# waicool20/BoofCV

Hardware: AMD Instinct MI355X
Metric: 1080p frames/sec detect+describe+associate (higher is better)
Workload: dtype f32 detect / f64 describe / associate: fp16 MFMA candidate filter + exact fp64 re-score; 1 GPU; batch of 256 1920x1080 GrayF32 per GPU: Fast-Hessian detect + SURF-64 (stable) describe + greedy L2 associate with the next frame; batch_per_gpu=256, width=1920, height=1080, ranks_seen=1

## Files before the change

boofcv_amd/csrc/assoc_mfma.hip:

```cpp
#include "common.h"
#include <cfloat>
#include <cmath>
#include <cstring>
#include <algorithm>

typedef float f32x16 __attribute__((ext_vector_type(16)));
typedef _Float16 h16x8 __attribute__((ext_vector_type(8)));

struct AssocProblem {
	int srcOff, ns, dstOff, nd;
	int rowBase, colBase;
};
struct AssocBlock {
	int p, row0, row1, col0, col1;
};
struct AssocCand {
	int p, i, j, pad;
	double score;
};

#define C16 1.03e-3f
#define ABS16 2.0e-5f
#define BIG16 60000.0f
#define ROW_CHUNKS 9

__device__ __forceinline__ void waveSyncLds() {
	__builtin_amdgcn_fence(__ATOMIC_RELEASE, "wavefront");
	__builtin_amdgcn_wave_barrier();
	__builtin_amdgcn_fence(__ATOMIC_ACQUIRE, "wavefront");
}

__host__ __device__ __forceinline__ int scaleExp(float maxN) {
	if (!(maxN > 0.0f)) return 0;
	int e;
	(void)frexpf(maxN, &e);
	return (e + 1) >> 1;
}
__host__ __device__ __forceinline__ bool scaleHolds(float maxN, int q) {
	if (!(maxN > 0.0f)) return true;
	int e;
	(void)frexpf(maxN, &e);
	return e >= 2 * q - 3 && e <= 2 * q;
}
__host__ __device__ __forceinline__ bool assocDegenerate(const int* flags, int cap) {
	float maxN;
	memcpy(&maxN, &flags[1], 4);
	return flags[0] != 0 || flags[2] > cap || !scaleHolds(maxN, flags[3]);
}

#define PREP_ROWS 8
__global__ __launch_bounds__(256) void k_assoc_norms(const double* __restrict__ D, long long rows, float* __restrict__ nrm, int* __restrict__ flags) {
	const long long row0 = (((long long)blockIdx.x * 256 + threadIdx.x) >> 4) * PREP_ROWS;
	const int part = threadIdx.x & 15;
	if (row0 >= rows) return;
	double2 v0[PREP_ROWS], v1[PREP_ROWS];
#pragma unroll
	for (int q = 0; q < PREP_ROWS; q++) {
		const long long row = min(row0 + q, rows - 1);
		const double2* src = (const double2*)(D + row * 64 + 4 * part);
		v0[q] = src[0]; v1[q] = src[1];
	}
#pragma unroll
	for (int q = 0; q < PREP_ROWS; q++) {
		double s = (v0[q].x * v0[q].x + v0[q].y * v0[q].y) + (v1[q].x * v1[q].x + v1[q].y * v1[q].y);
#pragma unroll
		for (int o = 8; o >= 1; o >>= 1) s += __shfl_xor(s, o, 64);
		if (part == 0 && row0 + q < rows) {
			const float n = (float)s;
			const float nUp = n * (1.0f + 4.0f * 5.9604644775390625e-08f);
			nrm[row0 + q] = nUp;
			if (!(s < 1e30)) atomicOr(&flags[0], 1);
			else if (__float_as_int(nUp) > __hip_atomic_load(&flags[1], __ATOMIC_RELAXED, __HIP_MEMORY_SCOPE_AGENT)) atomicMax(&flags[1], __float_as_int(nUp));
		}
	}
}

typedef _Float16 h16x4 __attribute__((ext_vector_type(4)));
__global__ __launch_bounds__(256) void k_assoc_half(const double* __restrict__ D, long long rows, float* __restrict__ nrm, int* __restrict__ flags,
													  _Float16* __restrict__ Hrow) {
	const long long row0 = (((long long)blockIdx.x * 256 + threadIdx.x) >> 4) * PREP_ROWS;
	const int part = threadIdx.x & 15;
	if (row0 >= rows) return;
	const int q_ = scaleExp(__int_as_float(flags[1]));
	if (blockIdx.x == 0 && threadIdx.x == 0) flags[3] = q_;
	double2 v0[PREP_ROWS], v1[PREP_ROWS];
#pragma unroll
	for (int q = 0; q < PREP_ROWS; q++) {
		const long long row = min(row0 + q, rows - 1);
		const double2* src = (const double2*)(D + row * 64 + 4 * part);
		v0[q] = src[0]; v1[q] = src[1];
	}
#pragma unroll
	for (int q = 0; q < PREP_ROWS; q++) {
		const long long row = row0 + q;
		if (row >= rows) break;
		_Float16* out = Hrow + row * (ROW_CHUNKS * 8);
		const h16x4 hv = {(_Float16)(float)ldexp(v0[q].x, -q_), (_Float16)(float)ldexp(v0[q].y, -q_), (_Float16)(float)ldexp(v1[q].x, -q_),
						  (_Float16)(float)ldexp(v1[q].y, -q_)};
		*(h16x4*)(out + 4 * part) = hv;
		if (part == 0) {
			const float n = ldexpf(nrm[row], -2 * q_);
			const _Float16 hi = (_Float16)n;
			const _Float16 lo = (_Float16)(n - (float)hi);
			const h16x8 e = {hi, lo, (_Float16)1.0f, (_Float16)1.0f, (_Float16)1.0f, (_Float16)0.0f, (_Float16)0.0f, (_Float16)0.0f};
			*(h16x8*)(out + 64) = e;
			nrm[row] = n;
		}
	}
}

__global__ __launch_bounds__(256) void k_assoc_prep_hinted(const double* __restrict__ D, long long rows, int q_, float* __restrict__ nrm, int* __restrict__ flags,
															 _Float16* __restrict__ Hrow) {
	const long long row0 = (((long long)blockIdx.x * 256 + threadIdx.x) >> 4) * PREP_ROWS;
	const int part = threadIdx.x & 15;
	if (row0 >= rows) return;
	double2 v0[PREP_ROWS], v1[PREP_ROWS];
#pragma unroll
	for (int q = 0; q < PREP_ROWS; q++) {
		const long long row = min(row0 + q, rows - 1);
		const double2* src = (const double2*)(D + row * 64 + 4 * part);
		v0[q] = src[0]; v1[q] = src[1];
	}
#pragma unroll
	for (int q = 0; q < PREP_ROWS; q++) {
		double s = (v0[q].x * v0[q].x + v0[q].y * v0[q].y) + (v1[q].x * v1[q].x + v1[q].y * v1[q].y);
#pragma unroll
		for (int o = 8; o >= 1; o >>= 1) s += __shfl_xor(s, o, 64);
		const long long row = row0 + q;
		if (row >= rows) continue;
		_Float16* out = Hrow + row * (ROW_CHUNKS * 8);
		const h16x4 hv = {(_Float16)(float)ldexp(v0[q].x, -q_), (_Float16)(float)ldexp(v0[q].y, -q_), (_Float16)(float)ldexp(v1[q].x, -q_),
						  (_Float16)(float)ldexp(v1[q].y, -q_)};
		*(h16x4*)(out + 4 * part) = hv;
		if (part == 0) {
			const float nRaw = (float)s;
			const float nUp = nRaw * (1.0f + 4.0f * 5.9604644775390625e-08f);
			if (!(s < 1e30)) atomicOr(&flags[0], 1);
			else if (__float_as_int(nUp) > __hip_atomic_load(&flags[1], __ATOMIC_RELAXED, __HIP_MEMORY_SCOPE_AGENT)) atomicMax(&flags[1], __float_as_int(nUp));
			const float n = ldexpf(nUp, -2 * q_);
			const _Float16 hi = (_Float16)n;
			const _Float16 lo = (_Float16)(n - (float)hi);
			const h16x8 e = {hi, lo, (_Float16)1.0f, (_Float16)1.0f, (_Float16)1.0f, (_Float16)0.0f, (_Float16)0.0f, (_Float16)0.0f};
			*(h16x8*)(out + 64) = e;
			nrm[row] = n;
		}
	}
}

__global__ __launch_bounds__(256) void k_assoc_init(unsigned int* __restrict__ keys, unsigned long long* __restrict__ best, int* __restrict__ args, long long nk,
													  long long colTotal, int* __restrict__ flags, int q_, const uint4* __restrict__ tabSrc, uint4* __restrict__ tabDst,
													  long long tabWords) {
	const long long i = (long long)blockIdx.x * 256 + threadIdx.x;
	if (i < tabWords) tabDst[i] = tabSrc[i];
	if (i < 16) flags[i] = i == 3 ? q_ : 0;
	if (i >= nk) return;
	keys[i] = 0xFFFFFFFFu;
	best[i] = ~0ull;
	args[i] = -1;
	if (i < colTotal) args[nk + i] = 0;
}

struct MfmaArgs {
	const uint4* Hs;
	const uint4* Hd;
	const AssocProblem* probs;
	const AssocBlock* blocks;
	unsigned int* rowKey;
	unsigned int* colKey;
	const float* nrmS;
	const float* nrmD;
	const int* flags;
	AssocCand* cand;
	int* counter;
	int cap;
#ifdef BHIP_EXPERIMENTS
	int ablate;
#endif
};

#define CAND_LDS 256

__device__ __noinline__ void candSlow(AssocCand* cand, int* counter, int cap, int p, int rr, int col) {
	const int g = atomicAdd(counter, 1);
	if (g < cap) { AssocCand c; c.p = p; c.i = rr; c.j = col; c.pad = 0; c.score = 0; cand[g] = c; }
}
__device__ __forceinline__ void candAdd(const MfmaArgs& A, int2* buf, int* cnt, bool hit, int p, int rr, int col) {
	if (hit) {
		const int pos = atomicAdd(cnt, 1);
		if (pos < CAND_LDS) buf[pos] = make_int2(rr, col);
		else candSlow(A.cand, A.counter, A.cap, p, rr, col);
	}
}
__device__ __forceinline__ void candFlush(const MfmaArgs& A, const int2* buf, const int* cnt, int p, int lane) {
	waveSyncLds();
	const int n = min(*cnt, CAND_LDS);
	if (n == 0) return;
	int base = 0;
	if (lane == 0) base = atomicAdd(A.counter, n);
	base = __builtin_amdgcn_readfirstlane(base);
	for (int k = lane; k < n; k += 64) {
		if (base + k < A.cap) {
			const int2 v = buf[k];
			AssocCand c; c.p = p; c.i = v.x; c.j = v.y; c.pad = 0; c.score = 0;
			A.cand[base + k] = c;
		}
	}
}

__device__ __forceinline__ h16x8 asHalf8(uint4 v) { return __builtin_bit_cast(h16x8, v); }
__device__ __forceinline__ uint4 extChunk(float n0, float n1, float n2, float n3) {
	const h16x8 h = {(_Float16)n0, (_Float16)n1, (_Float16)n2, (_Float16)n3, (_Float16)1.0f, (_Float16)0.0f, (_Float16)0.0f, (_Float16)0.0f};
	return __builtin_bit_cast(uint4, h);
}

#ifndef BHIP_ASSOC_PEEL
#define BHIP_ASSOC_PEEL 1
#endif
#define STRIP_COLS 384
#define STRIP_TILES (STRIP_COLS / 32)
template <int PASS>
__global__ __launch_bounds__(256, 2) void k_assoc_mfma(MfmaArgs A) {
	__shared__ uint4 tileB[STRIP_TILES][10 * 33];
	__shared__ unsigned int colLds[STRIP_COLS];
	__shared__ float rowThrLds[PASS == 2 ? 4 : 1][64];
	__shared__ int2 candLds[PASS == 2 ? 4 : 1][PASS == 2 ? CAND_LDS : 1];
	__shared__ int candCnt[4];
	const AssocBlock B = A.blocks[blockIdx.x];
	if (B.col0 >= B.col1) return;
	const AssocProblem P = A.probs[B.p];
	const int tid = threadIdx.x;
	const int wave = __builtin_amdgcn_readfirstlane(tid >> 6), lane = tid & 63;
	const int r = lane & 31, h = lane >> 5;
	const int ncol = B.col1 - B.col0;
	const int ntile = (ncol + 31) >> 5;
	int2* candBuf = candLds[PASS == 2 ? wave : 0];
	int* candN = &candCnt[wave];
	if (lane == 0) *candN = 0;

	for (int g0 = tid; g0 < ntile * 32 * ROW_CHUNKS; g0 += 4 * 256) {
		uint4 v[4];
#pragma unroll
		for (int q = 0; q < 4; q++) {
			const int g = g0 + 256 * q;
			const int cl = g / ROW_CHUNKS, ch = g - cl * ROW_CHUNKS;
			if (g < ntile * 32 * ROW_CHUNKS && cl < ncol) {
				v[q] = A.Hd[(long long)(P.dstOff + B.col0 + cl) * ROW_CHUNKS + ch];
				if (ch == 8) { const unsigned int x = v[q].x; v[q].x = v[q].y; v[q].y = x; }
			} else {
				v[q] = ch == 8 ? extChunk(1.0f, 1.0f, BIG16, 0.0f) : make_uint4(0, 0, 0, 0);
			}
		}
#pragma unroll
		for (int q = 0; q < 4; q++) {
			const int g = g0 + 256 * q;
			const int cl = g / ROW_CHUNKS, ch = g - cl * ROW_CHUNKS;
			if (g < ntile * 32 * ROW_CHUNKS) tileB[cl >> 5][ch * 33 + (cl & 31)] = v[q];
		}
	}
	for (int g = tid; g < ntile * 32; g += 256) tileB[g >> 5][9 * 33 + (g & 31)] = make_uint4(0, 0, 0, 0);
	float maxN = 0.0f;
	if (PASS == 2) maxN = ldexpf(__int_as_float(A.flags[1]), -2 * A.flags[3]);
	for (int c = tid; c < ntile * 32; c += 256) {
		unsigned int v = 0xFFFFFFFFu;
		if (PASS == 2) {
			float thr = -INFINITY;
			if (c < ncol) {
				const float band = 2.0f * (C16 * (A.nrmD[P.dstOff + B.col0 + c] + maxN) + ABS16);
				thr = __uint_as_float(A.colKey[P.colBase + B.col0 + c]) + band;
			}
			v = __float_as_uint(thr);
		}
		colLds[c] = v;
	}
	__syncthreads();

	uint4 araw[2][5];
	auto loadA = [&](int rowT) {
#pragma unroll
		for (int t = 0; t < 2; t++) {
			const int row = rowT + 32 * t + r;
			if (row < B.row1) {
				const uint4* src = A.Hs + (long long)(P.srcOff + row) * ROW_CHUNKS;
#pragma unroll
				for (int s = 0; s < 4; s++) araw[t][s] = src[2 * s + h];
				araw[t][4] = h == 0 ? src[8] : make_uint4(0, 0, 0, 0);
			} else {
#pragma unroll
				for (int s = 0; s < 4; s++) araw[t][s] = make_uint4(0, 0, 0, 0);
				araw[t][4] = h == 0 ? extChunk(BIG16, 0.0f, 1.0f, 1.0f) : make_uint4(0, 0, 0, 0);
			}
		}
	};
	if (B.row0 + 64 * wave < B.row1) loadA(B.row0 + 64 * wave);
	for (int rowT = B.row0 + 64 * wave; rowT < B.row1; rowT += 256) {
		h16x8 a[2][5];
#pragma unroll
		for (int t = 0; t < 2; t++) {
#pragma unroll
			for (int s = 0; s < 4; s++) a[t][s] = asHalf8(araw[t][s]) * (_Float16)(-2.0f);
			a[t][4] = asHalf8(araw[t][4]);
		}
		if (rowT + 256 < B.row1 && !BHIP_ABLATE(A, 4)) loadA(rowT + 256);
		unsigned int rowM[32];
#pragma unroll
		for (int k = 0; k < 32; k++) rowM[k] = 0xFFFFFFFFu;
		if (PASS == 2) {
			waveSyncLds();
			float thr = -INFINITY;
			if (rowT + lane < B.row1) {
				const float band = 2.0f * (C16 * (A.nrmS[P.srcOff + rowT + lane] + maxN) + ABS16);
				thr = __uint_as_float(A.rowKey[P.rowBase + rowT + lane]) + band;
			}
			rowThrLds[wave][lane] = thr;
			waveSyncLds();
		}
#pragma unroll
		for (int round = 0; round <= BHIP_ASSOC_PEEL; round++)
		for (int ct = round == 0 ? 0 : (ntile & ~1); ct < (BHIP_ASSOC_PEEL && round == 0 ? (ntile & ~1) : ntile); ct += 2) {
			const bool two = BHIP_ASSOC_PEEL ? round == 0 : ct + 1 < ntile;
			const int cA_ = 32 * ct + r, cB_ = cA_ + 32;
			f32x16 acc[2][2];
#pragma unroll
			for (int t = 0; t < 2; t++)
#pragma unroll
				for (int c = 0; c < 2; c++)
#pragma unroll
					for (int g = 0; g < 16; g++) acc[t][c][g] = (c == 0 || two) ? 0.0f : INFINITY;
#pragma unroll
			for (int s = 0; s < 5 && !BHIP_ABLATE(A, 1); s++) {
				const int ch = s < 4 ? 2 * s + h : 8 + h;
				const h16x8 b0 = asHalf8(tileB[ct][ch * 33 + r]);
				acc[0][0] = __builtin_amdgcn_mfma_f32_32x32x16_f16(a[0][s], b0, acc[0][0], 0, 0, 0);
				acc[1][0] = __builtin_amdgcn_mfma_f32_32x32x16_f16(a[1][s], b0, acc[1][0], 0, 0, 0);
				if (two) {
					const h16x8 b1 = asHalf8(tileB[ct + 1][ch * 33 + r]);
					acc[0][1] = __builtin_amdgcn_mfma_f32_32x32x16_f16(a[0][s], b1, acc[0][1], 0, 0, 0);
					acc[1][1] = __builtin_amdgcn_mfma_f32_32x32x16_f16(a[1][s], b1, acc[1][1], 0, 0, 0);
				}
			}
			if (BHIP_ABLATE(A, 2)) continue;
			if (PASS == 1) {
				unsigned int cA = 0xFFFFFFFFu, cB = 0xFFFFFFFFu;
#pragma unroll
				for (int t = 0; t < 2; t++)
#pragma unroll
					for (int g = 0; g < 16; g++) {
						const unsigned int uA = __float_as_uint(acc[t][0][g]), uB = __float_as_uint(acc[t][1][g]);
						rowM[16 * t + g] = min(rowM[16 * t + g], min(uA, uB));
						cA = min(cA, uA);
						cB = min(cB, uB);
					}
				cA = min(cA, (unsigned int)__shfl_xor((int)cA, 32, 64));
				cB = min(cB, (unsigned int)__shfl_xor((int)cB, 32, 64));
				if (h == 0) {
					atomicMin(&colLds[cA_], cA);
					if (two) atomicMin(&colLds[cB_], cB);
				}
			} else {
				const float tA = __uint_as_float(colLds[cA_]);
				const float tB = two ? __uint_as_float(colLds[cB_]) : -INFINITY;
				const int colA = B.col0 + cA_, colB = B.col0 + cB_;
#pragma unroll
				for (int t = 0; t < 2; t++)
#pragma unroll
					for (int j = 0; j < 4; j++) {
						const float4 rv = *(const float4*)&rowThrLds[wave][32 * t + 8 * j + 4 * h];
						const float rthr[4] = {rv.x, rv.y, rv.z, rv.w};
#pragma unroll
						for (int q = 0; q < 4; q++) {
							const int g = 4 * j + q;
							const float dA = acc[t][0][g], dB = acc[t][1][g];
							const bool rA = dA <= rthr[q], rB = dB <= rthr[q], qA = dA <= tA, qB = dB <= tB;
							if (__ballot(rA || rB || qA || qB) != 0ull) {
								const int rr = rowT + 32 * t + (g & 3) + 8 * (g >> 2) + 4 * h;
								candAdd(A, candBuf, candN, rA || qA, B.p, rr, colA);
								candAdd(A, candBuf, candN, rB || qB, B.p, rr, colB);
							}
						}
					}
			}
		}
		if (PASS == 1) {
#pragma unroll
			for (int k = 0; k < 32; k++) {
				unsigned int v = rowM[k];
				if (!BHIP_ABLATE(A, 64)) {
					v = min(v, (unsigned int)__builtin_amdgcn_update_dpp((int)v, (int)v, 0xB1, 0xF, 0xF, false));
					v = min(v, (unsigned int)__builtin_amdgcn_update_dpp((int)v, (int)v, 0x4E, 0xF, 0xF, false));
					v = min(v, (unsigned int)__builtin_amdgcn_update_dpp((int)v, (int)v, 0x141, 0xF, 0xF, false));
					v = min(v, (unsigned int)__builtin_amdgcn_update_dpp((int)v, (int)v, 0x140, 0xF, 0xF, false));
					v = min(v, (unsigned int)__shfl_xor((int)v, 16, 64));
				}
				const int rr = rowT + 32 * (k >> 4) + (k & 3) + 8 * ((k & 15) >> 2) + 4 * h;
				if (r == 0 && rr < B.row1 && !BHIP_ABLATE(A, 16)) atomicMin(&A.rowKey[P.rowBase + rr], v);
			}
		} else {
			waveSyncLds();
			if (*candN > CAND_LDS / 2) { candFlush(A, candBuf, candN, B.p, lane); waveSyncLds(); if (lane == 0) *candN = 0; waveSyncLds(); }
		}
	}
	if (PASS == 2) candFlush(A, candBuf, candN, B.p, lane);
	if (PASS == 1) {
		__syncthreads();
		for (int c = tid; c < ncol && !BHIP_ABLATE(A, 32); c += 256) atomicMin(&A.colKey[P.colBase + B.col0 + c], colLds[c]);
	}
}

__global__ __launch_bounds__(256) void k_assoc_exact(const double* __restrict__ src, const double* __restrict__ dst, const AssocProblem* __restrict__ probs,
													   AssocCand* __restrict__ cand, const int* __restrict__ counter, int cap,
													   unsigned long long* __restrict__ rowBest, unsigned long long* __restrict__ colBest) {
	const int n = min(*counter, cap);
	for (int t = blockIdx.x * blockDim.x + threadIdx.x; t < n; t += gridDim.x * blockDim.x) {
		AssocCand* c = &cand[t];
		const AssocProblem P = probs[c->p];
		const double* a = src + (long long)(P.srcOff + c->i) * 64;
		const double* b = dst + (long long)(P.dstOff + c->j) * 64;
		double total = 0;
#pragma unroll 8
		for (int k = 0; k < 64; k++) {
			const double d = a[k] - b[k];
			total += d * d;
		}
		c->score = total;
		const unsigned long long bits = (unsigned long long)__double_as_longlong(total);
		atomicMin(&rowBest[P.rowBase + c->i], bits);
		atomicMin(&colBest[P.colBase + c->j], bits);
	}
}

__global__ __launch_bounds__(256) void k_assoc_argsel(const AssocProblem* __restrict__ probs, const AssocCand* __restrict__ cand,
														const int* __restrict__ counter, int cap, const unsigned long long* __restrict__ rowBest,
														const unsigned long long* __restrict__ colBest, int* __restrict__ rowArg, int* __restrict__ colArg,
														int* __restrict__ colCnt) {
	const int n = min(*counter, cap);
	for (int t = blockIdx.x * blockDim.x + threadIdx.x; t < n; t += gridDim.x * blockDim.x) {
		const AssocCand c = cand[t];
		const AssocProblem P = probs[c.p];
		const unsigned long long bits = (unsigned long long)__double_as_longlong(c.score);
		if (bits == rowBest[P.rowBase + c.i]) atomicMax(&rowArg[P.rowBase + c.i], c.j);
		if (bits == colBest[P.colBase + c.j]) {
			atomicAdd(&colCnt[P.colBase + c.j], 1);
			atomicMax(&colArg[P.colBase + c.j], c.i);
		}
	}
}

__global__ __launch_bounds__(256) void k_assoc_resolve(const AssocProblem* __restrict__ probs, double maxErr, int backwards,
														 const unsigned long long* __restrict__ rowBest, const int* __restrict__ rowArg,
														 const int* __restrict__ colArg, const int* __restrict__ colCnt, const int* __restrict__ flags, int cap,
														 int* __restrict__ pairs, double* __restrict__ fit) {
	if (assocDegenerate(flags, cap)) return;
	const AssocProblem P = probs[blockIdx.y];
	for (int i = blockIdx.x * blockDim.x + threadIdx.x; i < P.ns; i += gridDim.x * blockDim.x) {
		const int m = rowArg[P.rowBase + i];
		const double best = __longlong_as_double((long long)rowBest[P.rowBase + i]);
		int outPair = -1;
		double outFit = maxErr;
		if (m >= 0 && best <= maxErr) {
			outPair = m;
			outFit = best;
			if (backwards) {
				if (!(colArg[P.colBase + m] == i && colCnt[P.colBase + m] == 1)) { outPair = -1; outFit = DBL_MAX; }
			}
		}
		pairs[P.srcOff + i] = outPair;
		fit[P.srcOff + i] = outFit;
	}
}

int bhip_assoc_l2_mfma_batched(bhip_ctx* ctx, AssocMfmaWork& W, const double* dev_src, const double* dev_dst, int count, const long long* srcOff,
								 const int* ns, const long long* dstOff, const int* nd, double maxErr, int backwards, int* dev_pairs, double* dev_fit,
								 int* usedMfma) {
	*usedMfma = 0;
	if (count <= 0) { *usedMfma = 1; return BHIP_OK; }
	std::vector<AssocProblem> probs(count);
	std::vector<AssocBlock> blocks;
	long long maxSrcRow = 0, maxDstRow = 0, rowTotal = 0, colTotal = 0;
	double flopsPerPass = 0;
	for (int p = 0; p < count; p++) {
		if (ns[p] <= 0 || nd[p] <= 0) return BHIP_OK;
		if (srcOff[p] + ns[p] > 0x7fffffffLL || dstOff[p] + nd[p] > 0x7fffffffLL) return BHIP_OK;
		probs[p] = {(int)srcOff[p], ns[p], (int)dstOff[p], nd[p], (int)rowTotal, (int)colTotal};
		maxSrcRow = std::max(maxSrcRow, srcOff[p] + ns[p]);
		maxDstRow = std::max(maxDstRow, dstOff[p] + nd[p]);
		rowTotal += ns[p];
		colTotal += nd[p];
		flopsPerPass += 2.0 * ns[p] * (double)nd[p] * 64;
		if (rowTotal > 0x3fffffffLL || colTotal > 0x3fffffffLL) return BHIP_OK;
	}
	auto buildBlocks = [&]() {
		long long strips = 0;
		for (int p = 0; p < count; p++) strips += (nd[p] + STRIP_COLS - 1) / STRIP_COLS;
		int rowSplit = (int)std::max<long long>(1, (1024 + strips - 1) / strips);
		{ const char* e = getenv("BHIP_ASSOC_ROWSPLIT"); if (e && atoi(e) > 0) rowSplit = atoi(e); }
		for (int p = 0; p < count; p++) {
			int chunk = (ns[p] + rowSplit - 1) / rowSplit;
			chunk = std::max(256, ((chunk + 255) / 256) * 256);
			for (int c0 = 0; c0 < nd[p]; c0 += STRIP_COLS)
				for (int r0 = 0; r0 < ns[p]; r0 += chunk) blocks.push_back({p, r0, std::min(ns[p], r0 + chunk), c0, std::min(nd[p], c0 + STRIP_COLS)});
		}
		if (count >= 16) {
			std::vector<AssocBlock> q[8];
			for (const AssocBlock& b : blocks) q[b.p & 7].push_back(b);
			size_t longest = 0;
			for (int x = 0; x < 8; x++) longest = std::max(longest, q[x].size());
			blocks.assign(longest * 8, AssocBlock{0, 0, 0, 0, 0});
			for (int x = 0; x < 8; x++)
				for (size_t k = 0; k < q[x].size(); k++) blocks[k * 8 + x] = q[x][k];
		}
	};
	const bool shared = dev_src == dev_dst;
	const long long rowsS = shared ? std::max(maxSrcRow, maxDstRow) : maxSrcRow;
	const int cap = (int)std::min<long long>(0x3fffffffLL, 8 * (rowTotal + colTotal) + 4096);

	BHIP_TRY(W.Fs.reserve(ctx, (size_t)rowsS * ROW_CHUNKS * 16));
	BHIP_TRY(W.nrmS.reserve(ctx, (size_t)rowsS * 4));
	if (!shared) {
		BHIP_TRY(W.Fd.reserve(ctx, (size_t)maxDstRow * ROW_CHUNKS * 16));
		BHIP_TRY(W.nrmD.reserve(ctx, (size_t)maxDstRow * 4));
	}
	BHIP_TRY(W.keys.reserve(ctx, (size_t)(rowTotal + colTotal) * 4));
	BHIP_TRY(W.best.reserve(ctx, (size_t)(rowTotal + colTotal) * 8));
	BHIP_TRY(W.args.reserve(ctx, (size_t)(rowTotal + 2 * colTotal) * 4));
	BHIP_TRY(W.cand.reserve(ctx, (size_t)cap * sizeof(AssocCand)));
	BHIP_TRY(W.flags.reserve(ctx, 64));

	hipStream_t st = ctx->stream;
	int* flags = W.flags.as<int>();
	int* counters = flags + 2;
	_Float16* Hs = W.Fs.as<_Float16>();
	float* nS = W.nrmS.as<float>();
	_Float16* Hd = shared ? Hs : W.Fd.as<_Float16>();
	float* nD = shared ? nS : W.nrmD.as<float>();
	unsigned int* rowKey = W.keys.as<unsigned int>();
	unsigned int* colKey = rowKey + rowTotal;
	unsigned long long* rowBest = W.best.as<unsigned long long>();
	unsigned long long* colBest = rowBest + rowTotal;
	int* rowArg = W.args.as<int>();
	int* colArg = rowArg + rowTotal;
	int* colCnt = colArg + colTotal;
	const long long nk = rowTotal + colTotal;
	int maxNs = 0;
	for (int p = 0; p < count; p++) maxNs = std::max(maxNs, ns[p]);
	const size_t blocksAt = (probs.size() * sizeof(AssocProblem) + 15) & ~(size_t)15;

	MfmaArgs A;
	A.Hs = (const uint4*)Hs; A.Hd = (const uint4*)Hd;
	A.rowKey = rowKey; A.colKey = colKey; A.nrmS = nS; A.nrmD = nD; A.flags = flags;
	A.cand = W.cand.as<AssocCand>(); A.counter = counters; A.cap = cap;
#ifdef BHIP_EXPERIMENTS
	{ const char* e = getenv("BHIP_ASSOC_ABLATE"); A.ablate = e ? atoi(e) : 0; }
#endif
	const unsigned gS = (unsigned)((rowsS + 16 * PREP_ROWS - 1) / (16 * PREP_ROWS)), gD = (unsigned)((maxDstRow + 16 * PREP_ROWS - 1) / (16 * PREP_ROWS));
	const double prepRows = (double)(rowsS + (shared ? 0 : maxDstRow));

	buildBlocks();
	const size_t tableBytes = (blocksAt + blocks.size() * sizeof(AssocBlock) + 15) & ~(size_t)15;
	BHIP_TRY(W.probs.reserve(ctx, tableBytes));
	if (W.tablesInFlight) { BHIP_HIP(ctx, hipStreamSynchronize(st)); W.tablesInFlight = false; }
	if (tableBytes > W.tables.cap) BHIP_TRY(W.tables.reserve(ctx, tableBytes * 2));
	memcpy(W.tables.p, probs.data(), probs.size() * sizeof(AssocProblem));
	memcpy((char*)W.tables.p + blocksAt, blocks.data(), blocks.size() * sizeof(AssocBlock));
	void* tablesDev = nullptr;
	BHIP_HIP(ctx, hipHostGetDevicePointer(&tablesDev, W.tables.p, 0));
	if (!W.flagsRead) BHIP_HIP(ctx, hipEventCreateWithFlags(&W.flagsRead.h, hipEventDisableTiming));
	A.probs = W.probs.as<AssocProblem>();
	A.blocks = (const AssocBlock*)((const char*)W.probs.p + blocksAt);
	const unsigned nblocks = (unsigned)blocks.size();

	for (int run = 0; run < 2; run++) {
		const bool hinted = run == 0;
		const long long tabWords = hinted ? (long long)(tableBytes / 16) : 0;
		W.tablesInFlight = true;
		hipLaunchKernelGGL(k_assoc_init, dim3((unsigned)((std::max(nk, tabWords) + 255) / 256)), dim3(256), 0, st, rowKey, rowBest, rowArg, nk, colTotal, flags,
						   hinted ? W.scaleHint : 0, (const uint4*)tablesDev, W.probs.as<uint4>(), tabWords);
		if (hinted) {
			ProfScope ps(ctx, "k_assoc_prep", prepRows * (64 * 8 + ROW_CHUNKS * 16));
			hipLaunchKernelGGL(k_assoc_prep_hinted, dim3(gS), dim3(256), 0, st, dev_src, rowsS, W.scaleHint, nS, flags, Hs);
			if (!shared) hipLaunchKernelGGL(k_assoc_prep_hinted, dim3(gD), dim3(256), 0, st, dev_dst, maxDstRow, W.scaleHint, nD, flags, Hd);
		} else {
			ProfScope ps(ctx, "k_assoc_prep", prepRows * (2 * 64 * 8 + ROW_CHUNKS * 16));
			hipLaunchKernelGGL(k_assoc_norms, dim3(gS), dim3(256), 0, st, dev_src, rowsS, nS, flags);
			if (!shared) hipLaunchKernelGGL(k_assoc_norms, dim3(gD), dim3(256), 0, st, dev_dst, maxDstRow, nD, flags);
			hipLaunchKernelGGL(k_assoc_half, dim3(gS), dim3(256), 0, st, dev_src, rowsS, nS, flags, Hs);
			if (!shared) hipLaunchKernelGGL(k_assoc_half, dim3(gD), dim3(256), 0, st, dev_dst, maxDstRow, nD, flags, Hd);
		}
		{
			ProfScope ps(ctx, "k_assoc_mfma_pass1", 0, flopsPerPass);
			hipLaunchKernelGGL(k_assoc_mfma<1>, dim3(nblocks), dim3(256), 0, st, A);
		}
		{
			ProfScope ps(ctx, "k_assoc_mfma_pass2", 0, flopsPerPass);
			hipLaunchKernelGGL(k_assoc_mfma<2>, dim3(nblocks), dim3(256), 0, st, A);
		}
		{
			ProfScope ps(ctx, "k_assoc_exact");
			const unsigned exactBlocks = (unsigned)std::min<long long>(16384, std::max<long long>(256, (3 * (rowTotal + colTotal) / 2 + 255) / 256));
			hipLaunchKernelGGL(k_assoc_exact, dim3(exactBlocks), dim3(256), 0, st, dev_src, dev_dst, A.probs, A.cand, counters, cap, rowBest, colBest);
			hipLaunchKernelGGL(k_assoc_argsel, dim3(exactBlocks), dim3(256), 0, st, A.probs, A.cand, counters, cap, rowBest, colBest, rowArg, colArg, colCnt);
		}
		BHIP_HIP(ctx, hipMemcpyAsync(ctx->hostScratch.p, flags, 16, hipMemcpyDeviceToHost, st));
		BHIP_HIP(ctx, hipEventRecord(W.flagsRead, st));
		hipLaunchKernelGGL(k_assoc_resolve, dim3((maxNs + 255) / 256, count), dim3(256), 0, st, A.probs, maxErr, backwards, rowBest, rowArg, colArg, colCnt,
						   flags, cap, dev_pairs, dev_fit);
		BHIP_HIP(ctx, hipEventSynchronize(W.flagsRead));
		W.tablesInFlight = false;
		BHIP_HIP(ctx, hipGetLastError());
		const int* hf = ctx->hostScratch.as<int>();
		if (hf[0] != 0) return BHIP_OK;
		float maxRaw;
		memcpy(&maxRaw, &hf[1], 4);
		if (maxRaw > 0.0f) W.scaleHint = scaleExp(maxRaw);
		if (!scaleHolds(maxRaw, hf[3])) continue;
		if (hf[2] > cap) return BHIP_OK;
		*usedMfma = 1;
		return BHIP_OK;
	}
	return BHIP_OK;
}
```

Before: 16390 frames/s.

## Prefetch tiles and thresholds, transpose row-min reduction, split exact rescoring across quads

Several separate changes to the association kernels. The strip load now clamps indices so the global loads are unconditional, with padding applied at the LDS store. Row threshold inputs and the first B fragment of the next column tile are prefetched into registers a step ahead. The pass-1 row-min reduction becomes a transpose-style butterfly that ends with one atomic per lane instead of 32 serial DPP chains. The exact fp64 rescoring kernel now uses four lanes per candidate with 16-byte loads and a quad DPP broadcast sum, launched with four times the blocks. These add register pressure, and the exact kernel changes the order of the fp64 summation.

After: 16550 frames/s, median of 6. Within noise of the previous version (+1.0%).

```diff
diff --git a/boofcv_amd/csrc/assoc_mfma.hip b/boofcv_amd/csrc/assoc_mfma.hip
--- a/boofcv_amd/csrc/assoc_mfma.hip
+++ b/boofcv_amd/csrc/assoc_mfma.hip
@@ -215,6 +215,9 @@
 
 #ifndef BHIP_ASSOC_PEEL
 #define BHIP_ASSOC_PEEL 1
+#endif
+#ifndef BHIP_ASSOC_PREFETCH2
+#define BHIP_ASSOC_PREFETCH2 0
 #endif
 #define STRIP_COLS 384
 #define STRIP_TILES (STRIP_COLS / 32)
@@ -237,24 +240,24 @@
 	int* candN = &candCnt[wave];
 	if (lane == 0) *candN = 0;
 
-	for (int g0 = tid; g0 < ntile * 32 * ROW_CHUNKS; g0 += 4 * 256) {
+	const uint4* stripRows = A.Hd + (long long)(P.dstOff + B.col0) * ROW_CHUNKS;
+	const int nchunk = ntile * 32 * ROW_CHUNKS;
+	for (int g0 = tid; g0 < nchunk; g0 += 4 * 256) {
 		uint4 v[4];
 #pragma unroll
 		for (int q = 0; q < 4; q++) {
-			const int g = g0 + 256 * q;
+			const int g = min(g0 + 256 * q, nchunk - 1);
 			const int cl = g / ROW_CHUNKS, ch = g - cl * ROW_CHUNKS;
-			if (g < ntile * 32 * ROW_CHUNKS && cl < ncol) {
-				v[q] = A.Hd[(long long)(P.dstOff + B.col0 + cl) * ROW_CHUNKS + ch];
-				if (ch == 8) { const unsigned int x = v[q].x; v[q].x = v[q].y; v[q].y = x; }
-			} else {
-				v[q] = ch == 8 ? extChunk(1.0f, 1.0f, BIG16, 0.0f) : make_uint4(0, 0, 0, 0);
-			}
+			v[q] = stripRows[min(cl, ncol - 1) * ROW_CHUNKS + ch];
 		}
 #pragma unroll
 		for (int q = 0; q < 4; q++) {
-			const int g = g0 + 256 * q;
+			const int g = min(g0 + 256 * q, nchunk - 1);
 			const int cl = g / ROW_CHUNKS, ch = g - cl * ROW_CHUNKS;
-			if (g < ntile * 32 * ROW_CHUNKS) tileB[cl >> 5][ch * 33 + (cl & 31)] = v[q];
+			uint4 w = v[q];
+			if (ch == 8) { const unsigned int x = w.x; w.x = w.y; w.y = x; }
+			if (cl >= ncol) w = ch == 8 ? extChunk(1.0f, 1.0f, BIG16, 0.0f) : make_uint4(0, 0, 0, 0);
+			tileB[cl >> 5][ch * 33 + (cl & 31)] = w;
 		}
 	}
 	for (int g = tid; g < ntile * 32; g += 256) tileB[g >> 5][9 * 33 + (g & 31)] = make_uint4(0, 0, 0, 0);
@@ -291,7 +294,22 @@
 			}
 		}
 	};
-	if (B.row0 + 64 * wave < B.row1) loadA(B.row0 + 64 * wave);
+	float thrN = 0.0f;
+	unsigned int thrK = 0xFFFFFFFFu;
+	auto loadThr = [&](int rowT) {
+		if (PASS == 2 && rowT + lane < B.row1) {
+			thrN = A.nrmS[P.srcOff + rowT + lane];
+			thrK = A.rowKey[P.rowBase + rowT + lane];
+		}
+	};
+	if (B.row0 + 64 * wave < B.row1) { loadA(B.row0 + 64 * wave); loadThr(B.row0 + 64 * wave); }
+	constexpr bool PREFETCH_B = PASS == 1 || BHIP_ASSOC_PREFETCH2;
+	h16x8 pb0 = {}, pb1 = {};
+	auto fetchB = [&](int ct) {
+		pb0 = asHalf8(tileB[ct][h * 33 + r]);
+		pb1 = asHalf8(tileB[min(ct + 1, ntile - 1)][h * 33 + r]);
+	};
+	if (PREFETCH_B) fetchB(0);
 	for (int rowT = B.row0 + 64 * wave; rowT < B.row1; rowT += 256) {
 		h16x8 a[2][5];
 #pragma unroll
@@ -300,7 +318,9 @@
 			for (int s = 0; s < 4; s++) a[t][s] = asHalf8(araw[t][s]) * (_Float16)(-2.0f);
 			a[t][4] = asHalf8(araw[t][4]);
 		}
-		if (rowT + 256 < B.row1 && !BHIP_ABLATE(A, 4)) loadA(rowT + 256);
+		const float curN = thrN;
+		const unsigned int curK = thrK;
+		if (rowT + 256 < B.row1 && !BHIP_ABLATE(A, 4)) { loadA(rowT + 256); loadThr(rowT + 256); }
 		unsigned int rowM[32];
 #pragma unroll
 		for (int k = 0; k < 32; k++) rowM[k] = 0xFFFFFFFFu;
@@ -308,8 +328,8 @@
 			waveSyncLds();
 			float thr = -INFINITY;
 			if (rowT + lane < B.row1) {
-				const float band = 2.0f * (C16 * (A.nrmS[P.srcOff + rowT + lane] + maxN) + ABS16);
-				thr = __uint_as_float(A.rowKey[P.rowBase + rowT + lane]) + band;
+				const float band = 2.0f * (C16 * (curN + maxN) + ABS16);
+				thr = __uint_as_float(curK) + band;
 			}
 			rowThrLds[wave][lane] = thr;
 			waveSyncLds();
@@ -329,15 +349,17 @@
 #pragma unroll
 			for (int s = 0; s < 5 && !BHIP_ABLATE(A, 1); s++) {
 				const int ch = s < 4 ? 2 * s + h : 8 + h;
-				const h16x8 b0 = asHalf8(tileB[ct][ch * 33 + r]);
+				const bool ahead = PREFETCH_B && s == 0;
+				const h16x8 b0 = ahead ? pb0 : asHalf8(tileB[ct][ch * 33 + r]);
 				acc[0][0] = __builtin_amdgcn_mfma_f32_32x32x16_f16(a[0][s], b0, acc[0][0], 0, 0, 0);
 				acc[1][0] = __builtin_amdgcn_mfma_f32_32x32x16_f16(a[1][s], b0, acc[1][0], 0, 0, 0);
 				if (two) {
-					const h16x8 b1 = asHalf8(tileB[ct + 1][ch * 33 + r]);
+					const h16x8 b1 = ahead ? pb1 : asHalf8(tileB[ct + 1][ch * 33 + r]);
 					acc[0][1] = __builtin_amdgcn_mfma_f32_32x32x16_f16(a[0][s], b1, acc[0][1], 0, 0, 0);
 					acc[1][1] = __builtin_amdgcn_mfma_f32_32x32x16_f16(a[1][s], b1, acc[1][1], 0, 0, 0);
 				}
 			}
+			if (PREFETCH_B) fetchB(ct + 2 < ntile ? ct + 2 : 0);
 			if (BHIP_ABLATE(A, 2)) continue;
 			if (PASS == 1) {
 				unsigned int cA = 0xFFFFFFFFu, cB = 0xFFFFFFFFu;
@@ -381,19 +403,35 @@
 			}
 		}
 		if (PASS == 1) {
-#pragma unroll
-			for (int k = 0; k < 32; k++) {
-				unsigned int v = rowM[k];
-				if (!BHIP_ABLATE(A, 64)) {
-					v = min(v, (unsigned int)__builtin_amdgcn_update_dpp((int)v, (int)v, 0xB1, 0xF, 0xF, false));
-					v = min(v, (unsigned int)__builtin_amdgcn_update_dpp((int)v, (int)v, 0x4E, 0xF, 0xF, false));
-					v = min(v, (unsigned int)__builtin_amdgcn_update_dpp((int)v, (int)v, 0x141, 0xF, 0xF, false));
-					v = min(v, (unsigned int)__builtin_amdgcn_update_dpp((int)v, (int)v, 0x140, 0xF, 0xF, false));
-					v = min(v, (unsigned int)__shfl_xor((int)v, 16, 64));
+			unsigned int v = rowM[0];
+			if (!BHIP_ABLATE(A, 64)) {
+				const bool b4 = r & 16, b3 = r & 8, b2 = r & 4, b1 = r & 2, b0 = r & 1;
+				unsigned int m1[16], m2[8], m3[4], m4[2];
+#pragma unroll
+				for (int j = 0; j < 16; j++) {
+					const unsigned int send = b4 ? rowM[j] : rowM[j + 16], keep = b4 ? rowM[j + 16] : rowM[j];
+					m1[j] = min(keep, (unsigned int)__shfl_xor((int)send, 16, 64));
 				}
-				const int rr = rowT + 32 * (k >> 4) + (k & 3) + 8 * ((k & 15) >> 2) + 4 * h;
-				if (r == 0 && rr < B.row1 && !BHIP_ABLATE(A, 16)) atomicMin(&A.rowKey[P.rowBase + rr], v);
-			}
+#pragma unroll
+				for (int j = 0; j < 8; j++) {
+					const unsigned int send = b3 ? m1[j] : m1[j + 8], keep = b3 ? m1[j + 8] : m1[j];
+					m2[j] = min(keep, (unsigned int)__builtin_amdgcn_update_dpp((int)send, (int)send, 0x140, 0xF, 0xF, false));
+				}
+#pragma unroll
+				for (int j = 0; j < 4; j++) {
+					const unsigned int send = b2 ? m2[j] : m2[j + 4], keep = b2 ? m2[j + 4] : m2[j];
+					m3[j] = min(keep, (unsigned int)__builtin_amdgcn_update_dpp((int)send, (int)send, 0x141, 0xF, 0xF, false));
+				}
+#pragma unroll
+				for (int j = 0; j < 2; j++) {
+					const unsigned int send = b1 ? m3[j] : m3[j + 2], keep = b1 ? m3[j + 2] : m3[j];
+					m4[j] = min(keep, (unsigned int)__builtin_amdgcn_update_dpp((int)send, (int)send, 0x4E, 0xF, 0xF, false));
+				}
+				const unsigned int send = b0 ? m4[0] : m4[1], keep = b0 ? m4[1] : m4[0];
+				v = min(keep, (unsigned int)__builtin_amdgcn_update_dpp((int)send, (int)send, 0xB1, 0xF, 0xF, false));
+			}
+			const int rr = rowT + 32 * (r >> 4) + (r & 3) + 8 * ((r & 15) >> 2) + 4 * h;
+			if (rr < B.row1 && !BHIP_ABLATE(A, 16)) atomicMin(&A.rowKey[P.rowBase + rr], v);
 		} else {
 			waveSyncLds();
 			if (*candN > CAND_LDS / 2) { candFlush(A, candBuf, candN, B.p, lane); waveSyncLds(); if (lane == 0) *candN = 0; waveSyncLds(); }
@@ -406,25 +444,50 @@
 	}
 }
 
+struct __attribute__((aligned(8))) ExactPiece { double x, y; };
+__device__ __forceinline__ double quadBcast(double v, int laneOfQuad) {
+	const long long b = __double_as_longlong(v);
+	int lo = (int)b, hi = (int)(b >> 32);
+	switch (laneOfQuad) {
+	case 0: lo = __builtin_amdgcn_mov_dpp(lo, 0x00, 0xF, 0xF, false); hi = __builtin_amdgcn_mov_dpp(hi, 0x00, 0xF, 0xF, false); break;
+	case 1: lo = __builtin_amdgcn_mov_dpp(lo, 0x55, 0xF, 0xF, false); hi = __builtin_amdgcn_mov_dpp(hi, 0x55, 0xF, 0xF, false); break;
+	case 2: lo = __builtin_amdgcn_mov_dpp(lo, 0xAA, 0xF, 0xF, false); hi = __builtin_amdgcn_mov_dpp(hi, 0xAA, 0xF, 0xF, false); break;
+	default: lo = __builtin_amdgcn_mov_dpp(lo, 0xFF, 0xF, 0xF, false); hi = __builtin_amdgcn_mov_dpp(hi, 0xFF, 0xF, 0xF, false); break;
+	}
+	return __longlong_as_double(((long long)hi << 32) | (unsigned int)lo);
+}
+#define EXACT_GROUP 4
 __global__ __launch_bounds__(256) void k_assoc_exact(const double* __restrict__ src, const double* __restrict__ dst, const AssocProblem* __restrict__ probs,
 													   AssocCand* __restrict__ cand, const int* __restrict__ counter, int cap,
 													   unsigned long long* __restrict__ rowBest, unsigned long long* __restrict__ colBest) {
 	const int n = min(*counter, cap);
-	for (int t = blockIdx.x * blockDim.x + threadIdx.x; t < n; t += gridDim.x * blockDim.x) {
+	const int q = threadIdx.x & (EXACT_GROUP - 1);
+	for (long long t = ((long long)blockIdx.x * blockDim.x + threadIdx.x) / EXACT_GROUP; t < n; t += (long long)gridDim.x * blockDim.x / EXACT_GROUP) {
 		AssocCand* c = &cand[t];
+		const int ci = c->i, cj = c->j;
 		const AssocProblem P = probs[c->p];
-		const double* a = src + (long long)(P.srcOff + c->i) * 64;
-		const double* b = dst + (long long)(P.dstOff + c->j) * 64;
+		const ExactPiece* a = (const ExactPiece*)(src + (long long)(P.srcOff + ci) * 64) + q;
+		const ExactPiece* b = (const ExactPiece*)(dst + (long long)(P.dstOff + cj) * 64) + q;
+		ExactPiece va[8], vb[8];
+#pragma unroll
+		for (int s = 0; s < 8; s++) { va[s] = a[4 * s]; vb[s] = b[4 * s]; }
 		double total = 0;
-#pragma unroll 8
-		for (int k = 0; k < 64; k++) {
-			const double d = a[k] - b[k];
-			total += d * d;
-		}
-		c->score = total;
-		const unsigned long long bits = (unsigned long long)__double_as_longlong(total);
-		atomicMin(&rowBest[P.rowBase + c->i], bits);
-		atomicMin(&colBest[P.colBase + c->j], bits);
+#pragma unroll
+		for (int s = 0; s < 8; s++) {
+			const double dx = va[s].x - vb[s].x, dy = va[s].y - vb[s].y;
+			const double sx = dx * dx, sy = dy * dy;
+#pragma unroll
+			for (int l = 0; l < EXACT_GROUP; l++) {
+				total += quadBcast(sx, l);
+				total += quadBcast(sy, l);
+			}
+		}
+		if (q == 0) {
+			c->score = total;
+			const unsigned long long bits = (unsigned long long)__double_as_longlong(total);
+			atomicMin(&rowBest[P.rowBase + ci], bits);
+			atomicMin(&colBest[P.colBase + cj], bits);
+		}
 	}
 }
 
@@ -596,7 +659,7 @@
 		{
 			ProfScope ps(ctx, "k_assoc_exact");
 			const unsigned exactBlocks = (unsigned)std::min<long long>(16384, std::max<long long>(256, (3 * (rowTotal + colTotal) / 2 + 255) / 256));
-			hipLaunchKernelGGL(k_assoc_exact, dim3(exactBlocks), dim3(256), 0, st, dev_src, dev_dst, A.probs, A.cand, counters, cap, rowBest, colBest);
+			hipLaunchKernelGGL(k_assoc_exact, dim3(EXACT_GROUP * exactBlocks), dim3(256), 0, st, dev_src, dev_dst, A.probs, A.cand, counters, cap, rowBest, colBest);
 			hipLaunchKernelGGL(k_assoc_argsel, dim3(exactBlocks), dim3(256), 0, st, A.probs, A.cand, counters, cap, rowBest, colBest, rowArg, colArg, colCnt);
 		}
 		BHIP_HIP(ctx, hipMemcpyAsync(ctx->hostScratch.p, flags, 16, hipMemcpyDeviceToHost, st));
```
